# KevinSpevak/openVO

Measured on AMD Instinct MI355X. Metric: stereo frame-pairs/sec (1280x720), higher is better.
Workload: dtype int16

## Files before the change

### openvo_amd/csrc/sgbm.hip

```cpp
#include "vo_internal.h"
#include <stdlib.h>
#include <algorithm>
#include <type_traits>

typedef short s16x2 __attribute__((ext_vector_type(2)));
typedef unsigned short u16x2 __attribute__((ext_vector_type(2)));

#define MAXC 0x7FFF
#define MAXC2 0x7FFF7FFFu
#define D2_EMPTY 0x7FFFFFFF

__device__ __forceinline__ s16x2 as_s(uint32_t v) { return __builtin_bit_cast(s16x2, v); }
__device__ __forceinline__ uint32_t as_u(s16x2 v) { return __builtin_bit_cast(uint32_t, v); }
__device__ __forceinline__ uint32_t pk_min(uint32_t a, uint32_t b) { return as_u(__builtin_elementwise_min(as_s(a), as_s(b))); }
__device__ __forceinline__ uint32_t pk_max(uint32_t a, uint32_t b) { return as_u(__builtin_elementwise_max(as_s(a), as_s(b))); }
__device__ __forceinline__ uint32_t pk_add(uint32_t a, uint32_t b) { return as_u(as_s(a) + as_s(b)); }
__device__ __forceinline__ uint32_t pk_sub(uint32_t a, uint32_t b) { return as_u(as_s(a) - as_s(b)); }
__device__ __forceinline__ uint32_t pk_add_sat(uint32_t a, uint32_t b) { return as_u(__builtin_elementwise_add_sat(as_s(a), as_s(b))); }
__device__ __forceinline__ uint32_t pk_sub_sat_u(uint32_t a, uint32_t b)
{
    return __builtin_bit_cast(uint32_t, __builtin_elementwise_sub_sat(__builtin_bit_cast(u16x2, a), __builtin_bit_cast(u16x2, b)));
}
__device__ __forceinline__ uint32_t pk_shr2(uint32_t a)
{
// ... 23 lines not shown
};

__device__ __forceinline__ int chan_val(const uint8_t* img, int W, int H, int x, int y, int c, int ft)
{
    if (x <= 0 || x >= W - 1) return ft;
    const uint8_t* r0 = img + (size_t)y * W;
    if (c == 1) return r0[x];
    const uint8_t* rn = y > 0 ? r0 - W : r0;
    const uint8_t* rs = y < H - 1 ? r0 + W : r0;
    int g = (r0[x + 1] - r0[x - 1]) * 2 + rn[x + 1] - rn[x - 1] + rs[x + 1] - rs[x - 1];
    return min(max(g, -ft), ft) + ft;
}

__device__ __forceinline__ void chan_bounds(const uint8_t* img, int W, int H, int x, int y, int c, int ft,
                                            int& v, int& lo, int& hi)
{
    v = chan_val(img, W, H, x, y, c, ft);
    int vl = x > 0 ? (v + chan_val(img, W, H, x - 1, y, c, ft)) / 2 : v;
    int vr = x < W - 1 ? (v + chan_val(img, W, H, x + 1, y, c, ft)) / 2 : v;
    lo = min(min(vl, vr), v);
    hi = max(max(vl, vr), v);
}

__global__ void k_sgbm_planes(const uint8_t* __restrict__ L, const uint8_t* __restrict__ R, int W, int H,
                              int ft, uint32_t* __restrict__ PL, uint32_t* __restrict__ PR, int* __restrict__ d2key,
                              int* __restrict__ sw_ctl, int sw_ctl_words, uint32_t* __restrict__ c_dummy, int dummy_words, uint32_t P2_2,
                              uint8_t* __restrict__ keepL, uint8_t* __restrict__ keepR)
{
    const int x = blockIdx.x * blockDim.x + threadIdx.x;
    for (int y = blockIdx.y; y < H; y += gridDim.y) {
    if (y == 1 && blockIdx.x == 0 && (int)threadIdx.x < dummy_words) c_dummy[threadIdx.x] = P2_2;
    if (y == 0 && blockIdx.x == 0)
        for (int i = threadIdx.x; i < sw_ctl_words; i += blockDim.x) sw_ctl[i] = 0;
    if (x >= W) return;
    size_t i = (size_t)y * W + x, plane = (size_t)W * H;
    if (keepL) { keepL[i] = L[i]; keepR[i] = R[i]; }
    if (d2key) d2key[i] = D2_EMPTY;
    for (int c = 0; c < 2; c++) {
        int v, lo, hi;
        chan_bounds(L, W, H, x, y, c, ft, v, lo, hi);
        PL[i * 2 + c] = (uint32_t)v | ((uint32_t)lo << 8) | ((uint32_t)hi << 16);
        int v1 = 0, lo1 = 0, hi1 = 0;
        chan_bounds(R, W, H, x, y, c, ft, v, lo, hi);
        if (x > 0) chan_bounds(R, W, H, x - 1, y, c, ft, v1, lo1, hi1);
        PR[(size_t)(c * 3 + 0) * plane + i] = (uint32_t)v | ((uint32_t)v1 << 16);
        PR[(size_t)(c * 3 + 1) * plane + i] = (uint32_t)lo | ((uint32_t)lo1 << 16);
        PR[(size_t)(c * 3 + 2) * plane + i] = (uint32_t)hi | ((uint32_t)hi1 << 16);
    }
    }
}

// ... 16 lines not shown
        if (c == 1) m = (m >> 2) & 0x3FFF3FFFu;
        acc = pk_add(acc, m);
    }
    return acc;
}

__device__ __forceinline__ uint32_t bt_regs(uint32_t lw0, uint32_t lw1, const uint32_t* V)
{
    uint32_t acc = 0;
#pragma unroll
    for (int c = 0; c < 2; c++) {
        const uint32_t lw = c ? lw1 : lw0;
        const uint32_t U = pk_rep(lw & 255), U0 = pk_rep((lw >> 8) & 255), U1 = pk_rep((lw >> 16) & 255);
        const uint32_t c0 = pk_sub_sat_u(U, V[c * 3 + 2]) | pk_sub_sat_u(V[c * 3 + 1], U);
        const uint32_t c1 = pk_sub_sat_u(V[c * 3 + 0], U1) | pk_sub_sat_u(U0, V[c * 3 + 0]);
        uint32_t m = pk_min(c0, c1);
        if (c == 1) m = pk_shr2(m);
        acc = pk_add(acc, m);
    }
    return acc;
}

template <int XT, int SW2>
__global__ void __launch_bounds__(128) k_sgbm_cost_sweep(const uint32_t* __restrict__ PL, const uint32_t* __restrict__ PR,
                                                        SgbmGeom g, int TY, int16_t* __restrict__ C)
{
    constexpr int WIN = 2 * SW2 + 1, NC = XT + 2 * SW2;
    constexpr bool RING_REGS = WIN <= 5;
    extern __shared__ uint32_t s_ring[];
    uint32_t ringv[RING_REGS ? WIN : 1][XT];
    uint32_t* const ring = s_ring + (size_t)(threadIdx.x >> 6) * WIN * XT * 64 + (threadIdx.x & 63);
    const int lane = threadIdx.x & 63, wv = threadIdx.x >> 6;
    const int dpl = threadIdx.x;
    const bool pad = 2 * dpl >= g.D;
    const int gx = (g.W1 + XT - 1) / XT, total = gx * ((g.H + TY - 1) / TY);
    const int chunk = (total + 7) >> 3, tile = (int)(blockIdx.x & 7) * chunk + (int)(blockIdx.x >> 3);
    if (tile >= total) return;
    const int tbx = tile % gx, tby = tile / gx;
    const int xa = tbx * XT, ya = tby * TY;
    const size_t plane = (size_t)g.W * g.H;
    const int yend = min(ya + TY, g.H);
    const int nrows = (yend - ya) + 2 * SW2;
    const int lane0_d = 2 * 64 * wv;
    const int krun = min(lane, NC - 1);
    const int xrun = min(max(xa - SW2 + krun, 0), g.W1 - 1) + g.minX1;
    const int prun = max(xrun - g.minD - lane0_d, 0);
    const int pown = max(-g.minD - 2 * (pad ? 0 : dpl), -(1 << 28));

    uint32_t acc[XT];
// ... 148 lines not shown
                if (rr >= WIN) acc[j] = pk_sub(acc[j], ringv[slot][j]);
                acc[j] = pk_add(acc[j], s);
                ringv[slot][j] = s;
            } else {
                uint32_t* cell = ring + (size_t)(slot * XT + j) * 64;
                if (rr >= WIN) acc[j] = pk_sub(acc[j], *cell);
                acc[j] = pk_add(acc[j], s);
                *cell = s;
            }
        }
        if (rr >= WIN - 1) {
            const int y = ya + rr - (WIN - 1);
#pragma unroll
            for (int j = 0; j < XT; j++) {
                const int x1 = xa + j;
                if (x1 < g.W1 && 2 * dpl < g.Dp)
                    *(uint32_t*)(C + ((size_t)y * g.W1 + x1) * g.Dp + 2 * dpl) = pad ? MAXC2 : acc[j];
            }
        }
    }
    }
}

__global__ void k_sgbm_cost_generic(const uint32_t* __restrict__ PL, const uint32_t* __restrict__ PR,
                                    SgbmGeom g, int16_t* __restrict__ C)
{
    const int dpl = threadIdx.x;
    if (2 * dpl >= g.Dp) return;
    const bool pad = 2 * dpl >= g.D;
    const int dp = pad ? 0 : dpl;
    const int x1 = blockIdx.x, y = blockIdx.y;
    const size_t plane = (size_t)g.W * g.H;
    const int pbase = g.minX1 - g.minD - 2 * dp;
    uint32_t acc = pk_rep(g.P2);
    for (int j = -g.SW2; j <= g.SW2; j++) {
        int r = min(max(y + j, 0), g.H - 1);
        for (int i = -g.SW2; i <= g.SW2; i++) {
            int xe = min(max(x1 + i, 0), g.W1 - 1);
            acc = pk_add(acc, bt_pair(PL, PR, plane, g.W, r, xe + g.minX1, xe + pbase));
        }
    }
    *(uint32_t*)(C + ((size_t)y * g.W1 + x1) * g.Dp + 2 * dpl) = pad ? MAXC2 : acc;
}

template <int NP>
struct LV { uint32_t r[NP]; };

template <int NP>
__device__ __forceinline__ LV<NP> lv_load(const int16_t* p)
// ... 1008 lines not shown
static int ensure_S(vo_ctx* ctx, int vols)
{
    if (ctx->ws->S_vols >= vols) return VO_OK;
    if (ctx->ws->S) (void)hipFree(ctx->ws->S);
    ctx->ws->S = nullptr; ctx->ws->S_vols = 0;
    VO_HIP(ctx, hipMalloc((void**)&ctx->ws->S, ctx->vol_cells * sizeof(int16_t) * vols + 256));
    ctx->ws->S_vols = vols;
    return VO_OK;
}

static_assert(VO_MAX_SWEEP_GROUP == DG_MAXJOBS, "include/vo355.h promises what one sweep launch carries");
struct SweepGroup {
    typedef int (*Launch)(vo_ctx*, const DiagJobs&, const SgbmGeom&);
    typedef int (*WeLaunch)(vo_ctx*, const WeJobs&, int, const SgbmGeom&);
    struct Member {
        int engine;
        hipStream_t stream;
        FrameSlot* f;
        int w, h;
        SgbmGeom g;
        DiagJob job;
        WeJob we;
        PostJob post;
    };
    Launch launch = nullptr;
    WeLaunch we_launch = nullptr;
    int nstrips = 0;
    int n = 0;
    hipStream_t lane = nullptr;
    Member m[DG_MAXJOBS];
    bool want_defer = false, did_defer = false;
    Member cand;
    Launch cand_launch = nullptr;
    WeLaunch cand_we_launch = nullptr;
    int cand_nstrips = 0;
};

template <int NP>
static int we2_launch_jobs(vo_ctx* ctx, const WeJobs& jobs, int n, const SgbmGeom& g)
{
    const dim3 grid(n, div_up(div_up(g.H, 4), 2));
    if (g.D != g.Dp) hipLaunchKernelGGL((k_sgbm_we2<NP, true>), grid, dim3(256), 0, ctx->stream, jobs, g, ctx->dump);
    else hipLaunchKernelGGL((k_sgbm_we2<NP, false>), grid, dim3(256), 0, ctx->stream, jobs, g, ctx->dump);
    VO_CHECK_LAUNCH(ctx);
    return VO_OK;
}
// ... 53 lines not shown
            G->cand_nstrips = jobs.nstrips;
            G->did_defer = true;
            return VO_OK;
        }
    }
    return diag_launch_jobs<NP, PAD, NWC, REV, WTA>(ctx, jobs, g);
}

template <int NP, bool REV, bool WTA>
static int launch_diag(vo_ctx* ctx, const SgbmGeom& g, const int16_t* in1, int16_t* sout, int* ctl)
{
    const bool pad = g.D != g.Dp;
    if constexpr (NP <= 4) {
        const int nwc = ctx->tune_diag_nwc ? ctx->tune_diag_nwc : (ctx->cur_engine >= 0 ? 11 : 7);
        if (nwc == 15)
            return pad ? launch_diag_k<NP, true, 15, REV, WTA>(ctx, g, in1, sout, ctl) : launch_diag_k<NP, false, 15, REV, WTA>(ctx, g, in1, sout, ctl);
        if (nwc == 11)
            return pad ? launch_diag_k<NP, true, 11, REV, WTA>(ctx, g, in1, sout, ctl) : launch_diag_k<NP, false, 11, REV, WTA>(ctx, g, in1, sout, ctl);
    }

    return pad ? launch_diag_k<NP, true, 7, REV, WTA>(ctx, g, in1, sout, ctl) : launch_diag_k<NP, false, 7, REV, WTA>(ctx, g, in1, sout, ctl);
}

template <int NP>
static int launch_agg(vo_ctx* ctx, const SgbmGeom& g, const PathPlan& plan, size_t vol)
{
    const bool pad = g.D != g.Dp;
    const bool hh = plan.n_dirs == 8;
    int rc;
    if (g.ur < 100) {
        if ((rc = ensure_S(ctx, 3))) return rc;
        int16_t* const Swe = ctx->ws->S;
        int16_t* const Srev = ctx->ws->S + vol;
        int16_t* const ck = ctx->ws->S + 2 * vol;
        int* const ctlA = ctx->ws->sw_ctl;
        int* const ctlB = ctx->ws->sw_ctl + ctx->sw_ctl_words / 2;
        const bool cut = g.W1 % 16 == 0 && g.W1 >= 32 && !(ctx->tune_diag_dbg & 8);
        SweepGroup* const G = ctx->grp;
        const bool defer_we = cut && G && G->want_defer && !hh && !(ctx->tune_diag_dbg & 16);
        if (G) G->cand_we_launch = nullptr;
        {
            StageTimer t(ctx, VO_T_SGBM_AGG, defer_we ? 0 : 1);
            if (ctx->tune_diag_dbg & 8) {
            } else if (cut) {
                WeJobs wj;
                memset(&wj, 0, sizeof(wj));
                wj.j[0].C = ctx->ws->C; wj.j[0].Swe = Swe; wj.j[0].ckpt = ck;
                if (defer_we) {
                    G->cand.we = wj.j[0];
                    G->cand_we_launch = &we2_launch_jobs<NP>;
                } else if ((rc = we2_launch_jobs<NP>(ctx, wj, 1, g))) return rc;
            } else if (g.W1 % 8 == 0 && g.W1 >= 16) {
                const int nw = div_up(g.H, 4);
                if (pad) hipLaunchKernelGGL((k_sgbm_we<NP, true>), dim3(div_up(nw, 4)), dim3(256), 0, ctx->stream, ctx->ws->C, Swe, ck, g, ctx->dump);
                else hipLaunchKernelGGL((k_sgbm_we<NP, false>), dim3(div_up(nw, 4)), dim3(256), 0, ctx->stream, ctx->ws->C, Swe, ck, g, ctx->dump);
            } else {
                PathPlan pp = plan;
                pp.n_dirs = 1;
                pp.sx[0] = 1; pp.sy[0] = 0; pp.nlines[0] = g.H;
                pp.first_wave[0] = 0;
                for (int k = 0; k < VO_MAX_DIRS; k++) pp.first_wave[k + 1] = div_up(g.H, 4);
                for (int k = 1; k < VO_MAX_DIRS; k++) pp.sx[k] = pp.sy[k] = pp.nlines[k] = 0;
// ... 25 lines not shown
        else hipLaunchKernelGGL((k_sgbm_paths<NP, PF, false>), dim3(div_up(nwaves, 4)), dim3(256), 0, ctx->stream, ctx->ws->C, ctx->ws->S, vol, g, plan, ctx->dump);
        VO_CHECK_LAUNCH(ctx);
    }
    {
        StageTimer t(ctx, VO_T_SGBM_WTA);
        const size_t sh = (size_t)16 * g.Dp * sizeof(int16_t);
        const long long npix = (long long)g.W1 * g.H;
        hipLaunchKernelGGL((k_sgbm_wta<NP>), dim3((unsigned)((npix + 15) / 16)), dim3(256), sh, ctx->stream, ctx->ws->S, vol, plan.n_dirs,
                           g, ctx->ws->disp_tmp, ctx->ws->ccl_size);
        VO_CHECK_LAUNCH(ctx);
    }
    ctx->last_paths = plan.n_dirs;
    ctx->last_schedule = VO_SCHED_UNFUSED;
    return VO_OK;
}

static int sgbm_run_impl(vo_ctx* ctx, FrameSlot& f, int w, int h, const uint8_t* srcL, const uint8_t* srcR);
static int sgbm_post(vo_ctx* ctx, FrameSlot& f, int w, int h, const SgbmGeom& g);
static PostJob post_job(const vo_ctx* ctx, const FrameSlot& f);
static int sgbm_post_launch(vo_ctx* ctx, const PostJobs& jobs, int n, const SgbmGeom& g, bool rows);
static uint32_t pk_rep_host(int v) { return (uint32_t)(v & 0xFFFF) * 0x00010001u; }
static int post_rows_per_block(int w) { return std::min(6, (int)(150 * 1024 / ((size_t)w * 6)) - 2); }

static int sgbm_run_done(vo_ctx* ctx)
{
    if (ctx->ws == &ctx->main_ws && ctx->ws->done) {
        VO_HIP(ctx, hipEventRecord(ctx->ws->done, ctx->stream));
        ctx->ws->done_valid = true;
        ctx->ws->done_on_engine0 = false;
        ctx->ws->done_lane = nullptr;
    }
    return VO_OK;
}

int sgbm_run(vo_ctx* ctx, FrameSlot& f, int w, int h, const uint8_t* srcL, const uint8_t* srcR, bool* deferred)
{
    int rc;
    if (deferred) *deferred = false;
    if (ctx->cur_engine < 0 && sweep_group_has_engine(ctx, 0) && (rc = sweep_group_close(ctx, VO_GRP_CONSUMER))) return rc;
    const bool shared = ctx->ws == &ctx->main_ws;
    if (shared && ctx->ws->done_valid && !(ctx->cur_engine == 0 && ctx->ws->done_on_engine0) && !(ctx->ws->done_lane && ctx->ws->done_lane == ctx->stream)) VO_HIP(ctx, hipStreamWaitEvent(ctx->stream, ctx->ws->done, 0));
    if (++ctx->sweep_gen_next <= 0) ctx->sweep_gen_next = 1;
    f.disp_gen = ctx->sweep_gen_next;
    const bool defer = deferred && ctx->cur_engine >= 0 && sweep_group_size(ctx) > 1 && ctx->sg.set && ctx->sg.ur < 100 && ctx->sg.mode == 0 &&
                       ctx->ws_alt[ctx->cur_engine].mid != nullptr;
    if (defer) {
        if (!ctx->grp) ctx->grp = new SweepGroup();
        ctx->grp->want_defer = true;
        ctx->grp->did_defer = false;
    }
    rc = sgbm_run_impl(ctx, f, w, h, srcL, srcR);
    if (defer) {
        SweepGroup* const G = ctx->grp;
        G->want_defer = false;
        if (!rc && G->did_defer) {
            G->did_defer = false;
            if (G->n > 0 && (G->n >= DG_MAXJOBS || G->launch != G->cand_launch || G->we_launch != G->cand_we_launch || G->nstrips != G->cand_nstrips ||
                             memcmp(&G->m[0].g, &G->cand.g, sizeof(SgbmGeom))) &&
                (rc = sweep_group_close(ctx, VO_GRP_OTHER)))
                return rc;
            SweepGroup::Member& m = G->m[G->n++];
            m = G->cand;
            m.engine = ctx->cur_engine; m.stream = ctx->stream; m.f = &f; m.w = w; m.h = h;
            if (G->n == 1) G->lane = stream_is_lane(ctx, ctx->stream) ? ctx->stream : nullptr;
            m.post = post_job(ctx, f);
            G->launch = G->cand_launch; G->we_launch = G->cand_we_launch; G->nstrips = G->cand_nstrips;
            f.in_group = true;
            *deferred = true;
            return VO_OK;
        }
    }
    if (int rcd = sgbm_run_done(ctx)) return rcd;
    return rc;
}

hipStream_t dense_stream(const vo_ctx* ctx, int engine)
{
    if (!lane_mode(ctx) || !ctx->sg.set || ctx->sg.ur >= 100 || ctx->sg.mode != 0) return ctx->la_stream[engine];
    const SweepGroup* const G = ctx->grp;
    return G && G->n > 0 && G->lane ? G->lane : ctx->lane[ctx->lane_next];
}

bool sweep_group_has_engine(const vo_ctx* ctx, int engine)
{
    if (ctx->grp)
        for (int i = 0; i < ctx->grp->n; i++)
            if (ctx->grp->m[i].engine == engine) return true;
    return false;
}
int sweep_group_members(const vo_ctx* ctx) { return ctx->grp ? ctx->grp->n : 0; }
void sweep_group_free(vo_ctx* ctx) { delete ctx->grp; ctx->grp = nullptr; }
// ... 61 lines not shown
    G->n = 0;
    for (int i = 0; i < n; i++) G->m[i].f->in_group = false;
    ctx->grp_closed[why]++;
    int rc = VO_OK;
    {
        MemberScope scope(ctx);
        SweepGroup::Member& last = G->m[n - 1];
        scope.enter(last.engine);
        hipStream_t const lane = G->lane;
        G->lane = nullptr;
        if (lane) {
            ctx->stream = lane;
            ctx->lane_next = lane == ctx->lane[0] ? 1 : 0;
        }
        DiagJobs jobs;
        WeJobs we;
        PostJobs post;
        memset(&jobs, 0, sizeof(jobs));
        memset(&we, 0, sizeof(we));
        memset(&post, 0, sizeof(post));
        jobs.n = n; jobs.nstrips = G->nstrips;
        jobs.j[0] = last.job; we.j[0] = last.we; post.j[0] = last.post;
        bool main_member = last.engine == 0;
        for (int i = 0; i + 1 < n && !rc; i++) {
            jobs.j[i + 1] = G->m[i].job; we.j[i + 1] = G->m[i].we; post.j[i + 1] = G->m[i].post;
            main_member |= G->m[i].engine == 0;
            const vo_ctx::SgbmWs& a = ctx->ws_alt[G->m[i].engine];
            if (lane && G->m[i].stream == lane) continue;
            if (!a.mid_valid || hipStreamWaitEvent(ctx->stream, a.mid, 0) != hipSuccess) rc = vo_fail(ctx, VO_E_HIP, "sweep group: waiting for a member's early stages failed");
        }
        if (!rc && G->we_launch) {
            StageTimer t(ctx, VO_T_SGBM_AGG, n);
            rc = G->we_launch(ctx, we, n, last.g);
        }
        if (!rc) {
            StageTimer t(ctx, VO_T_SGBM_WTA, n);
            rc = G->launch(ctx, jobs, last.g);
        }
        const bool post_here = post_rows_per_block(last.g.W) >= 1;
        if (!rc && post_here) {
            if (!(ctx->tune_diag_dbg & 32)) {
                StageTimer t(ctx, VO_T_SGBM_POST, n);
                rc = sgbm_post_launch(ctx, post, n, last.g, true);
            }
            if (!rc && main_member && ctx->main_ws.done) {
                if (hipEventRecord(ctx->main_ws.done, ctx->stream) == hipSuccess) { ctx->main_ws.done_valid = true; ctx->main_ws.done_on_engine0 = false; ctx->main_ws.done_lane = lane; }
// ... 58 lines not shown
    int maxX1 = w + (e.minD < 0 ? e.minD : 0);
    g.W1 = maxX1 - g.minX1;
    g.invalid16 = (e.minD - 1) * 16;
    const int n = w * h;
    if (g.W1 <= 0) {
        if (srcL) {
            VO_HIP(ctx, hipMemcpyAsync(f.left, srcL, (size_t)n, hipMemcpyDeviceToDevice, ctx->stream));
            VO_HIP(ctx, hipMemcpyAsync(f.right, srcR, (size_t)n, hipMemcpyDeviceToDevice, ctx->stream));
        }
        std::vector<int16_t> inv((size_t)n, (int16_t)g.invalid16);
        VO_HIP(ctx, hipMemcpyAsync(d_disp, inv.data(), (size_t)n * 2, hipMemcpyHostToDevice, ctx->stream));
        VO_HIP(ctx, hipStreamSynchronize(ctx->stream));
        ctx->last_cells = 0;
        return VO_OK;
    }
    const size_t vol = (size_t)g.W1 * h * g.Dp;
    if (vol > ctx->vol_cells || e.D > 256)
        return vo_fail(ctx, VO_E_CAP, "cost volume %zu cells exceeds the capacity given to vo_create (or D > 256)", vol);
    if (((size_t)g.W1 * h + 1) * g.Dp * 2 >= 0xFFFFFF00ull)
        return vo_fail(ctx, VO_E_CAP, "cost volume of %zu bytes exceeds the 4 GiB a volume kernel addresses", ((size_t)g.W1 * h + 1) * g.Dp * 2);
    const PathPlan plan = make_plan(g, e.mode);
    ctx->last_cells = (int64_t)g.W1 * h * g.D;
    {
        StageTimer t(ctx, VO_T_SGBM_COST);
        const int dbg = ctx->tune_diag_dbg;
        hipLaunchKernelGGL(k_sgbm_planes, dim3(div_up(w, 256), std::min(h, 128)), dim3(256), 0, ctx->stream, dL, dR, w, h, g.ftzero,
                           ctx->ws->planesL, ctx->ws->planesR, (g.ur >= 100 || post_rows_per_block(w) < 1) ? ctx->ws->ccl_size : nullptr, ctx->ws->sw_ctl, ctx->sw_ctl_words,
                           (uint32_t*)(ctx->ws->C + vol), g.Dp / 2, pk_rep_host(g.P2), srcL ? f.left : nullptr, srcL ? f.right : nullptr);
        const int bx = ((g.Dp / 2 + 63) / 64) * 64;
        const int TY = ctx->tune_sweep_ty;
        const int nw = bx / 64;
#define LAUNCH_SWEEP(XT, SW)                                                                                                   \
    hipLaunchKernelGGL((k_sgbm_cost_sweep<XT, SW>), dim3(8 * div_up(div_up(g.W1, XT) * div_up(h, TY), 8)), dim3(bx),            \
                       (size_t)nw * (((2 * SW + 1) <= 5 ? 0 : (2 * SW + 1) * XT * 64) + 12 * (64 + (XT + 2 * SW - 1) / 2)) * 4, ctx->stream, ctx->ws->planesL, ctx->ws->planesR, g, TY, ctx->ws->C)
        if (dbg & 4) {
        } else
        switch (g.SW2) {
            case 0: LAUNCH_SWEEP(8, 0); break;
            case 1: LAUNCH_SWEEP(8, 1); break;
            case 2: LAUNCH_SWEEP(8, 2); break;
            case 3: LAUNCH_SWEEP(8, 3); break;
            case 4: LAUNCH_SWEEP(8, 4); break;
            case 5: LAUNCH_SWEEP(8, 5); break;
            default:
                hipLaunchKernelGGL(k_sgbm_cost_generic, dim3(g.W1, h), dim3(bx), 0, ctx->stream, ctx->ws->planesL, ctx->ws->planesR, g, ctx->ws->C);
        }
#undef LAUNCH_SWEEP
        VO_CHECK_LAUNCH(ctx);
    }
    int rc;
    switch (g.Dp / 32) {
        case 1: rc = launch_agg<1>(ctx, g, plan, vol); break;
        case 2: rc = launch_agg<2>(ctx, g, plan, vol); break;
        case 3: rc = launch_agg<3>(ctx, g, plan, vol); break;
        case 4: rc = launch_agg<4>(ctx, g, plan, vol); break;
        case 5: rc = launch_agg<5>(ctx, g, plan, vol); break;
        case 6: rc = launch_agg<6>(ctx, g, plan, vol); break;
        case 7: rc = launch_agg<7>(ctx, g, plan, vol); break;
        default: rc = launch_agg<8>(ctx, g, plan, vol); break;
    }
    if (rc) return rc;
    if (ctx->grp && ctx->grp->did_defer) return VO_OK;
    return sgbm_post(ctx, f, w, h, g);
}

static PostJob post_job(const vo_ctx* ctx, const FrameSlot& f)
{
    PostJob j;
    j.aux0 = ctx->ws->rec; j.aux1 = ctx->ws->rec + (size_t)ctx->max_w * ctx->max_h + 64;
    j.dst = f.disp16;
    j.L = ctx->ws->ccl_label; j.runlen = ctx->ws->ccl_runlen; j.size = ctx->ws->ccl_size;
// ... 54 lines not shown
```

### openvo_amd/csrc/vo_ctx.hip

```cpp
#include <stdarg.h>
#include <stdlib.h>
#include "vo_internal.h"

int vo_fail(vo_ctx* ctx, int code, const char* fmt, ...)
{
    char buf[1024];
    va_list ap;
    va_start(ap, fmt);
    vsnprintf(buf, sizeof(buf), fmt, ap);
    va_end(ap);
    if (ctx) ctx->err = buf;
    return code;
}

static thread_local std::string g_create_err;
static int lanes_ensure(vo_ctx* ctx);

static const size_t ARENA_BASE = 4096;

static void* arena_take(vo_ctx* ctx, size_t bytes)
{
    const size_t need = (bytes + 63) & ~(size_t)63;
    if (ARENA_BASE + ctx->arena_off + need > ctx->pinned_bytes) return nullptr;
    void* p = (char*)ctx->pinned + ARENA_BASE + ctx->arena_off;
// ... 133 lines not shown
    int ndev = 0;
    hipError_t e = hipGetDeviceCount(&ndev);
    if (e != hipSuccess || ndev <= 0) {
        g_create_err = std::string("vo_create: no HIP device available (") + hipGetErrorString(e) +
                       "); libvo355 has no CPU fallback";
        return VO_E_HIP;
    }
    if (device_id < 0 || device_id >= ndev) { g_create_err = "vo_create: bad device id"; return VO_E_ARG; }
    vo_ctx* ctx = new vo_ctx();
    ctx->device = device_id;
    ctx->max_w = max_w; ctx->max_h = max_h; ctx->max_disp = max_disp; ctx->max_kp = max_kp;
    if ((e = hipSetDevice(device_id)) != hipSuccess) { g_create_err = hipGetErrorString(e); delete ctx; return VO_E_HIP; }
    hipDeviceProp_t prop;
    if (hipGetDeviceProperties(&prop, device_id) == hipSuccess) {
        char generic[96];
        snprintf(generic, sizeof(generic), "AMD GPU, %d CUs, %.0f GB", prop.multiProcessorCount, (double)prop.totalGlobalMem / 1e9);
        snprintf(ctx->devname, sizeof(ctx->devname), "%s (%s)", prop.name[0] ? prop.name : generic, prop.gcnArchName);
    }
    if ((e = hipStreamCreateWithFlags(&ctx->stream, hipStreamNonBlocking)) != hipSuccess) { g_create_err = hipGetErrorString(e); delete ctx; return VO_E_HIP; }
    if (const char* e8 = getenv("VO_ENGINES")) { int v = atoi(e8); if (v >= 1 && v <= vo_ctx::MAX_ENGINES) ctx->n_engines = v; }
    if (const char* eq = getenv("GPU_MAX_HW_QUEUES")) { int v = atoi(eq); if (v >= 1) ctx->hw_queues = v; }
    if (const char* eg = getenv("VO_SWEEP_GROUP")) { int v = atoi(eg); if (v >= 1 && v <= VO_MAX_SWEEP_GROUP) ctx->sweep_group_req = v; }
    if (const char* el = getenv("VO_GROUP_LANES")) ctx->lanes_on = atoi(el) != 0;
    if (lanes_ensure(ctx)) { g_create_err = "hipStreamCreate failed (lane streams)"; vo_destroy(ctx); return VO_E_HIP; }
    (void)hipEventCreate(&ctx->ev0);
    (void)hipEventCreate(&ctx->ev1);

    const size_t npx = (size_t)max_w * max_h;
    ctx->kp_cap = max_kp * 2 + 1024;
    for (int s = 0; s <= VO_NUM_SLOTS; s++) {
        FrameSlot& f = ctx->slots[s];
        DALLOC(f.left, npx); DALLOC(f.right, npx); DALLOC(f.disp16, npx);
        (void)hipEventCreateWithFlags(&f.ready, hipEventDisableTiming);
        DALLOC(f.kp_xy, (size_t)ctx->kp_cap * 2); DALLOC(f.kp_size, ctx->kp_cap); DALLOC(f.kp_angle, ctx->kp_cap);
        DALLOC(f.kp_resp, ctx->kp_cap); DALLOC(f.kp_oct, ctx->kp_cap); DALLOC(f.desc, (size_t)ctx->kp_cap * 32);
        DALLOC(f.mono_depth, ctx->kp_cap); DALLOC(f.mono_serial_dev, 16);
        DALLOC(f.kp_xyz, (size_t)ctx->kp_cap * 3); DALLOC(f.kp_disp, ctx->kp_cap); DALLOC(f.kp_rdesc, (size_t)ctx->kp_cap * 32);
        if (dev_zero(f.mono_serial_dev, 64) != hipSuccess) { g_create_err = "clearing a slot's depth serial failed"; vo_destroy(ctx); return VO_E_HIP; }
    }
    {
        FrameSlot& r = ctx->sparse_r;
        DALLOC(r.kp_xy, (size_t)ctx->kp_cap * 2); DALLOC(r.kp_size, ctx->kp_cap); DALLOC(r.kp_angle, ctx->kp_cap);
        DALLOC(r.kp_resp, ctx->kp_cap); DALLOC(r.kp_oct, ctx->kp_cap); DALLOC(r.desc, (size_t)ctx->kp_cap * 32);
        ctx->sp_main.l = &ctx->slots[VO_NUM_SLOTS]; ctx->sp_main.r = &r;
    }
    ctx->stage_bytes = npx * 3;
// ... 348 lines not shown
    return VO_OK;
}

extern "C" int vo_upload_mono(vo_ctx* ctx, int slot, const uint8_t* img, int w, int h, int channels)
{
    int rc = check_slot(ctx, slot);
    if (rc) return rc;
    if (!img || (channels != 1 && channels != 3)) return vo_fail(ctx, VO_E_ARG, "vo_upload_mono: bad argument");
    if (w > ctx->max_w || h > ctx->max_h || w < 16 || h < 16) return vo_fail(ctx, VO_E_CAP, "image %dx%d exceeds context %dx%d", w, h, ctx->max_w, ctx->max_h);
    VO_HIP(ctx, hipSetDevice(ctx->device));
    FrameSlot& f = ctx->slots[slot];
    if ((rc = slot_wait(ctx, f)) || (rc = slot_before_overwrite(ctx, f))) return rc;
    StageTimer t(ctx, VO_T_UPLOAD);
    if ((rc = ingest(ctx, 0, img, w, h, channels, 1, f.left, ctx->stage_in))) return rc;
    f.w = w; f.h = h; f.has_pair = true; f.has_disp = false; f.has_kp = false; f.kp_depth = false; f.sp_pending = false; f.n_kp = 0; f.kp_pending = false;
    return VO_OK;
}

extern "C" int vo_stage_pairs_alloc(vo_ctx* ctx, int n, int w, int h, int channels)
{
    if (!ctx || n <= 0 || (channels != 1 && channels != 3)) return vo_fail(ctx, VO_E_ARG, "vo_stage_pairs_alloc: bad argument");
    if (w > ctx->max_w || h > ctx->max_h || w < 16 || h < 16) return vo_fail(ctx, VO_E_CAP, "image %dx%d exceeds context", w, h);
    VO_HIP(ctx, hipSetDevice(ctx->device));
    if (ctx->staged) { (void)hipFree(ctx->staged); ctx->staged = nullptr; }
    ctx->staged_n = 0;
    const size_t per = (size_t)w * h * channels;
    VO_HIP(ctx, hipMalloc((void**)&ctx->staged, per * 2 * n));
    ctx->staged_n = n; ctx->staged_w = w; ctx->staged_h = h; ctx->staged_ch = channels;
    return VO_OK;
}

extern "C" int vo_stage_pair(vo_ctx* ctx, int index, const uint8_t* left, const uint8_t* right)
{
    if (!ctx || !left || !right || index < 0 || index >= ctx->staged_n) return vo_fail(ctx, VO_E_ARG, "vo_stage_pair: bad index");
    VO_HIP(ctx, hipSetDevice(ctx->device));
    const size_t per = (size_t)ctx->staged_w * ctx->staged_h * ctx->staged_ch;
    VO_HIP(ctx, hipMemcpyAsync(ctx->staged + per * 2 * index, left, per, hipMemcpyHostToDevice, ctx->stream));
    VO_HIP(ctx, hipMemcpyAsync(ctx->staged + per * (2 * index + 1), right, per, hipMemcpyHostToDevice, ctx->stream));
    VO_HIP(ctx, hipStreamSynchronize(ctx->stream));
    return VO_OK;
}

extern "C" int vo_load_staged_pair(vo_ctx* ctx, int slot, int index, int preprocessed)
{
    int rc = check_slot(ctx, slot);
    if (rc) return rc;
    if (index < 0 || index >= ctx->staged_n) return vo_fail(ctx, VO_E_ARG, "vo_load_staged_pair: bad index");
    VO_HIP(ctx, hipSetDevice(ctx->device));
    FrameSlot& f = ctx->slots[slot];
    const int w = ctx->staged_w, h = ctx->staged_h;
    const size_t per = (size_t)w * h * ctx->staged_ch;
    StageTimer t(ctx, VO_T_UPLOAD);
    if ((rc = slot_wait(ctx, f)) || (rc = slot_before_overwrite(ctx, f))) return rc;
    rc = ingest(ctx, 0, ctx->staged + per * 2 * index, w, h, ctx->staged_ch, preprocessed, f.left, ctx->stage_in, hipMemcpyDeviceToDevice);
    if (rc) return rc;
    rc = ingest(ctx, 1, ctx->staged + per * (2 * index + 1), w, h, ctx->staged_ch, preprocessed, f.right, ctx->stage_in, hipMemcpyDeviceToDevice);
    if (rc) return rc;
    f.w = w; f.h = h; f.has_pair = true; f.has_disp = false; f.has_kp = false; f.kp_depth = false; f.sp_pending = false; f.n_kp = 0; f.kp_pending = false;
    return VO_OK;
// ... 871 lines not shown
```

### openvo_amd/csrc/vo_internal.h

```cpp
#pragma once
#include <hip/hip_runtime.h>
#include <stdint.h>
#include <stdio.h>
#include <string.h>
#include <string>
#include <vector>
#include <deque>
#include <thread>
#include <mutex>
#include <condition_variable>
#include "../../include/vo355.h"

#define VO_ORB_LEVELS 8
#define VO_ORB_EDGE 31
#define VO_ORB_HALF_PATCH 15

struct SgbmEff {
    int minD, maxD, D, ur, d12, P1, P2, SW2, SH2, ftzero, minX1, maxX1, W1, invalid16;
    int speckleWindow, speckleRange, mode;
    bool set;
};

struct OrbLevel {
    int w, h;
// ... 63 lines not shown
struct MapSet {
    float* xyz = nullptr;
    uint8_t *desc = nullptr, *rdesc = nullptr;
    int32_t *oct = nullptr, *obs = nullptr, *last = nullptr;
};
struct LandmarkMap {
    bool used = false;
    int capacity = 0, n = 0, cur = 0, view_n = 0;
    int max_serial = -1;
    MapSet set[2];
    int32_t *view_src = nullptr, *d_q = nullptr, *d_t = nullptr;
    uint8_t *claimed = nullptr, *d_mask = nullptr;
    std::vector<uint8_t> seen;
};
void map_free(LandmarkMap& m);

struct vo_ctx {
    int device = 0;
    hipStream_t stream = nullptr;
    static const int MAX_ENGINES = 24;
    hipStream_t la_stream[MAX_ENGINES] = {};
    hipStream_t lane[2] = {nullptr, nullptr};
    bool lanes_on = true;
    bool lane_used = false;
    int lane_next = 0;
    int cur_engine = -1;
    int tune_stagger = -1;
    uint8_t* la_stage[MAX_ENGINES] = {};
    struct SgbmWs {
        uint32_t *planesL = nullptr, *planesR = nullptr;
        int16_t *C = nullptr, *S = nullptr, *disp_tmp = nullptr;
        int32_t *ccl_runlen = nullptr, *ccl_label = nullptr, *ccl_size = nullptr;
        int32_t* rec = nullptr;
        int S_vols = 0;
        uint64_t* sw_bnd = nullptr;
        size_t sw_bnd_bytes = 0;
        int* sw_ctl = nullptr;
        uint32_t sw_tag = 0;
        hipEvent_t done = nullptr;
        bool done_valid = false;
        bool done_on_engine0 = false;
        hipStream_t done_lane = nullptr;
        bool ready = false;
        OrbWs orb;
        uint8_t* pinned = nullptr;
        hipEvent_t h2d_done = nullptr;
// ... 233 lines not shown
{
    int few = VO_SWEEP_GROUP_FEW_QUEUES;
    if (ctx->lanes_on && few > ctx->n_engines / 2) few = ctx->n_engines >= 2 ? ctx->n_engines / 2 : 1;
    int b = ctx->sweep_group_req > 0 ? ctx->sweep_group_req : (ctx->hw_queues >= ctx->n_engines + 4 ? 1 : few);
    return b < ctx->n_engines ? b : ctx->n_engines;
}
static inline bool lane_mode(const vo_ctx* ctx) { return ctx->lanes_on && ctx->lane[0] && ctx->lane[1] && sweep_group_size(ctx) > 1; }
static inline int pose_stream_count(const vo_ctx* ctx)
{
    int n = ctx->n_pose_streams;
    if (!ctx->pose_streams_env && ctx->lane_used && lane_mode(ctx) && n > ctx->hw_queues - 3) n = ctx->hw_queues - 3 > 1 ? ctx->hw_queues - 3 : 1;
    return n;
}
static inline bool stream_is_lane(const vo_ctx* ctx, hipStream_t s) { return s && (s == ctx->lane[0] || s == ctx->lane[1]); }
static inline hipError_t engine_streams_sync(const vo_ctx* ctx)
{
    for (int k = 0; k < 2; k++)
        if (ctx->lane[k]) { const hipError_t e = hipStreamSynchronize(ctx->lane[k]); if (e != hipSuccess) return e; }
    for (int k = 0; k < vo_ctx::MAX_ENGINES; k++)
        if (ctx->la_stream[k]) { const hipError_t e = hipStreamSynchronize(ctx->la_stream[k]); if (e != hipSuccess) return e; }
    return hipSuccess;
}
int sweep_group_close(vo_ctx* ctx, int why);
int engine_behind_chain(vo_ctx* ctx, int engine);
int engine_enter(vo_ctx* ctx, int engine, hipStream_t target);
hipStream_t dense_stream(const vo_ctx* ctx, int engine);
bool sweep_group_has_engine(const vo_ctx* ctx, int engine);
int sweep_group_members(const vo_ctx* ctx);
void sweep_group_free(vo_ctx* ctx);
static inline int sweep_group_close_for(vo_ctx* ctx, const FrameSlot& f) { return f.in_group ? sweep_group_close(ctx, VO_GRP_CONSUMER) : VO_OK; }
int slot_health(vo_ctx* ctx, const FrameSlot& f, int slot);
int orb_prepare_tables(vo_ctx* ctx, int w, int h);
int orb_run(vo_ctx* ctx, FrameSlot* fs, const uint8_t* d_img, int img_stride, int w, int h,
            int nfeatures, int mask_mode, const int16_t* d_disp16, int disp_stride, int min_d16,
            int max_d16, const uint8_t* d_mask, int mask_stride);
#define VO_KNN_SPLITS 16
static inline size_t match_dist_bytes(int kp_cap)
{
    const size_t capq = ((size_t)kp_cap + 63) & ~(size_t)63;
    return capq * 8 + (size_t)VO_KNN_SPLITS * capq * 8 + (capq / 64 + 1) * 4 + capq * 4 + 256;
}
static inline uint32_t* match_colmin(int32_t* d_dist, int kp_cap)
{
    const size_t capq = ((size_t)kp_cap + 63) & ~(size_t)63;
    return (uint32_t*)((uint8_t*)d_dist + capq * 8 + (size_t)VO_KNN_SPLITS * capq * 8 + (capq / 64 + 1) * 4);
}
// ... 61 lines not shown
```

Baseline: 2182.

## Batch SGBM planes and cost-volume launches across sweep-group frames

The planes and cost-sweep kernels now take an array of per-frame jobs indexed by a grid dimension. When frames are deferred into a sweep group on a lane stream, each frame's front-end work is queued, then launched as one batched kernel pair once enough frames are pending or the group closes. This cuts per-frame launch count and lets several frames fill the GPU together. The cost is extra deferral bookkeeping, flush points in the staging APIs, and an abandon path for the group when a batched launch fails.

```diff
diff --git a/openvo_amd/csrc/sgbm.hip b/openvo_amd/csrc/sgbm.hip
--- a/openvo_amd/csrc/sgbm.hip
+++ b/openvo_amd/csrc/sgbm.hip
@@ -69,11 +69,29 @@
     hi = max(max(vl, vr), v);
 }
 
-__global__ void k_sgbm_planes(const uint8_t* __restrict__ L, const uint8_t* __restrict__ R, int W, int H,
-                              int ft, uint32_t* __restrict__ PL, uint32_t* __restrict__ PR, int* __restrict__ d2key,
-                              int* __restrict__ sw_ctl, int sw_ctl_words, uint32_t* __restrict__ c_dummy, int dummy_words, uint32_t P2_2,
-                              uint8_t* __restrict__ keepL, uint8_t* __restrict__ keepR)
-{
+struct FrontJob {
+    const uint8_t *L, *R;
+    uint32_t *planesL, *planesR;
+    int* d2key;
+    int* sw_ctl;
+    uint32_t* dummy;
+    uint8_t *keepL, *keepR;
+    int16_t* C;
+};
+struct FrontJobs { FrontJob j[VO_MAX_SWEEP_GROUP]; };
+
+__global__ void k_sgbm_planes(FrontJobs jobs, int W, int H, int ft, int sw_ctl_words, int dummy_words, uint32_t P2_2)
+{
+    const FrontJob& J = jobs.j[blockIdx.z];
+    const uint8_t* __restrict__ const L = J.L;
+    const uint8_t* __restrict__ const R = J.R;
+    uint32_t* __restrict__ const PL = J.planesL;
+    uint32_t* __restrict__ const PR = J.planesR;
+    int* __restrict__ const d2key = J.d2key;
+    int* __restrict__ const sw_ctl = J.sw_ctl;
+    uint32_t* __restrict__ const c_dummy = J.dummy;
+    uint8_t* __restrict__ const keepL = J.keepL;
+    uint8_t* __restrict__ const keepR = J.keepR;
     const int x = blockIdx.x * blockDim.x + threadIdx.x;
     for (int y = blockIdx.y; y < H; y += gridDim.y) {
     if (y == 1 && blockIdx.x == 0 && (int)threadIdx.x < dummy_words) c_dummy[threadIdx.x] = P2_2;
@@ -136,9 +154,12 @@
 }
 
 template <int XT, int SW2>
-__global__ void __launch_bounds__(128) k_sgbm_cost_sweep(const uint32_t* __restrict__ PL, const uint32_t* __restrict__ PR,
-                                                        SgbmGeom g, int TY, int16_t* __restrict__ C)
-{
+__global__ void __launch_bounds__(128) k_sgbm_cost_sweep(FrontJobs jobs, SgbmGeom g, int TY)
+{
+    const FrontJob& J = jobs.j[blockIdx.y];
+    const uint32_t* __restrict__ const PL = J.planesL;
+    const uint32_t* __restrict__ const PR = J.planesR;
+    int16_t* __restrict__ const C = J.C;
     constexpr int WIN = 2 * SW2 + 1, NC = XT + 2 * SW2;
     constexpr bool RING_REGS = WIN <= 5;
     extern __shared__ uint32_t s_ring[];
@@ -333,9 +354,12 @@
     }
 }
 
-__global__ void k_sgbm_cost_generic(const uint32_t* __restrict__ PL, const uint32_t* __restrict__ PR,
-                                    SgbmGeom g, int16_t* __restrict__ C)
-{
+__global__ void k_sgbm_cost_generic(FrontJobs jobs, SgbmGeom g)
+{
+    const FrontJob& J = jobs.j[blockIdx.z];
+    const uint32_t* __restrict__ const PL = J.planesL;
+    const uint32_t* __restrict__ const PR = J.planesR;
+    int16_t* __restrict__ const C = J.C;
     const int dpl = threadIdx.x;
     if (2 * dpl >= g.Dp) return;
     const bool pad = 2 * dpl >= g.D;
@@ -1390,6 +1414,8 @@
         DiagJob job;
         WeJob we;
         PostJob post;
+        FrontJob front;
+        bool front_pending;
     };
     Launch launch = nullptr;
     WeLaunch we_launch = nullptr;
@@ -1489,6 +1515,21 @@
     return pad ? launch_diag_k<NP, true, 7, REV, WTA>(ctx, g, in1, sout, ctl) : launch_diag_k<NP, false, 7, REV, WTA>(ctx, g, in1, sout, ctl);
 }
 
+static bool we2_geometry(const vo_ctx* ctx, const SgbmGeom& g) { return g.W1 % 16 == 0 && g.W1 >= 32 && !(ctx->tune_diag_dbg & 8); }
+
+static bool run_defers_we(const vo_ctx* ctx, const SgbmGeom& g, bool hh)
+{
+    const SweepGroup* const G = ctx->grp;
+    return G && G->want_defer && g.ur < 100 && g.W1 > 0 && we2_geometry(ctx, g) && !hh && !(ctx->tune_diag_dbg & 16);
+}
+
+static bool run_defers_front(const vo_ctx* ctx, const SgbmGeom& g, bool hh)
+{
+    if (ctx->front_batch < 2 || ctx->cur_engine < 0 || (ctx->tune_diag_dbg & 4) || !run_defers_we(ctx, g, hh)) return false;
+    if (!lane_mode(ctx) || !stream_is_lane(ctx, ctx->stream)) return false;
+    return ctx->grp->n == 0 || ctx->grp->lane == ctx->stream;
+}
+
 template <int NP>
 static int launch_agg(vo_ctx* ctx, const SgbmGeom& g, const PathPlan& plan, size_t vol)
 {
@@ -1502,9 +1543,9 @@
         int16_t* const ck = ctx->ws->S + 2 * vol;
         int* const ctlA = ctx->ws->sw_ctl;
         int* const ctlB = ctx->ws->sw_ctl + ctx->sw_ctl_words / 2;
-        const bool cut = g.W1 % 16 == 0 && g.W1 >= 32 && !(ctx->tune_diag_dbg & 8);
+        const bool cut = we2_geometry(ctx, g);
         SweepGroup* const G = ctx->grp;
-        const bool defer_we = cut && G && G->want_defer && !hh && !(ctx->tune_diag_dbg & 16);
+        const bool defer_we = run_defers_we(ctx, g, hh);
         if (G) G->cand_we_launch = nullptr;
         {
             StageTimer t(ctx, VO_T_SGBM_AGG, defer_we ? 0 : 1);
@@ -1576,6 +1617,80 @@
 static uint32_t pk_rep_host(int v) { return (uint32_t)(v & 0xFFFF) * 0x00010001u; }
 static int post_rows_per_block(int w) { return std::min(6, (int)(150 * 1024 / ((size_t)w * 6)) - 2); }
 
+static int front_launch(vo_ctx* ctx, const FrontJobs& jobs, int n, const SgbmGeom& g)
+{
+    const int w = g.W, h = g.H;
+    hipLaunchKernelGGL(k_sgbm_planes, dim3(div_up(w, 256), std::min(h, 128), n), dim3(256), 0, ctx->stream, jobs, w, h, g.ftzero,
+                       ctx->sw_ctl_words, g.Dp / 2, pk_rep_host(g.P2));
+    const int bx = ((g.Dp / 2 + 63) / 64) * 64;
+    const int TY = ctx->tune_sweep_ty;
+    const int nw = bx / 64;
+#define LAUNCH_SWEEP(XT, SW)                                                                                                   \
+    hipLaunchKernelGGL((k_sgbm_cost_sweep<XT, SW>), dim3(8 * div_up(div_up(g.W1, XT) * div_up(h, TY), 8), n), dim3(bx),         \
+                       (size_t)nw * (((2 * SW + 1) <= 5 ? 0 : (2 * SW + 1) * XT * 64) + 12 * (64 + (XT + 2 * SW - 1) / 2)) * 4, ctx->stream, jobs, g, TY)
+    if (ctx->tune_diag_dbg & 4) {
+    } else
+    switch (g.SW2) {
+        case 0: LAUNCH_SWEEP(8, 0); break;
+        case 1: LAUNCH_SWEEP(8, 1); break;
+        case 2: LAUNCH_SWEEP(8, 2); break;
+        case 3: LAUNCH_SWEEP(8, 3); break;
+        case 4: LAUNCH_SWEEP(8, 4); break;
+        case 5: LAUNCH_SWEEP(8, 5); break;
+        default:
+            hipLaunchKernelGGL(k_sgbm_cost_generic, dim3(g.W1, h, n), dim3(bx), 0, ctx->stream, jobs, g);
+    }
+#undef LAUNCH_SWEEP
+    VO_CHECK_LAUNCH(ctx);
+    return VO_OK;
+}
+
+static int sweep_group_launch_fronts(vo_ctx* ctx, SweepGroup* G, int n, hipStream_t lane)
+{
+    FrontJobs fj;
+    memset(&fj, 0, sizeof(fj));
+    int k = 0;
+    for (int i = 0; i < n; i++)
+        if (G->m[i].front_pending) { fj.j[k++] = G->m[i].front; G->m[i].front_pending = false; }
+    if (k == 0) return VO_OK;
+    hipStream_t const s0 = ctx->stream;
+    ctx->stream = lane;
+    int rc;
+    {
+        StageTimer t(ctx, VO_T_SGBM_COST, k);
+        rc = front_launch(ctx, fj, k, G->m[0].g);
+    }
+    ctx->stream = s0;
+    return rc;
+}
+
+static void sweep_group_abandon(vo_ctx* ctx)
+{
+    SweepGroup* const G = ctx->grp;
+    for (int i = 0; i < G->n; i++) {
+        FrameSlot& f = *G->m[i].f;
+        f.in_group = false; f.kp_pending = false; f.has_pair = false; f.has_disp = false;
+        if (f.counted && ctx->inflight > 0) ctx->inflight--;
+        f.counted = false;
+    }
+    G->n = 0;
+    G->lane = nullptr;
+}
+
+int sweep_group_flush_fronts(vo_ctx* ctx, bool wait)
+{
+    SweepGroup* const G = ctx->grp;
+    if (!G || G->n == 0 || !G->lane) return VO_OK;
+    bool any = false;
+    for (int i = 0; i < G->n; i++) any |= G->m[i].front_pending;
+    if (!any) return VO_OK;
+    (void)hipSetDevice(ctx->device);
+    hipStream_t const lane = G->lane;
+    if (int rc = sweep_group_launch_fronts(ctx, G, G->n, lane)) { sweep_group_abandon(ctx); return rc; }
+    if (wait) VO_HIP(ctx, hipStreamSynchronize(lane));
+    return VO_OK;
+}
+
 static int sgbm_run_done(vo_ctx* ctx)
 {
     if (ctx->ws == &ctx->main_ws && ctx->ws->done) {
@@ -1602,6 +1717,7 @@
         if (!ctx->grp) ctx->grp = new SweepGroup();
         ctx->grp->want_defer = true;
         ctx->grp->did_defer = false;
+        ctx->grp->cand.front_pending = false;
     }
     rc = sgbm_run_impl(ctx, f, w, h, srcL, srcR);
     if (defer) {
@@ -1621,6 +1737,12 @@
             G->launch = G->cand_launch; G->we_launch = G->cand_we_launch; G->nstrips = G->cand_nstrips;
             f.in_group = true;
             *deferred = true;
+            int pending = 0;
+            for (int i = 0; i < G->n; i++) pending += G->m[i].front_pending ? 1 : 0;
+            if (pending >= ctx->front_batch && G->lane && (rc = sweep_group_launch_fronts(ctx, G, G->n, G->lane))) {
+                sweep_group_abandon(ctx);
+                return rc;
+            }
             return VO_OK;
         }
     }
@@ -1728,6 +1850,7 @@
         jobs.n = n; jobs.nstrips = G->nstrips;
         jobs.j[0] = last.job; we.j[0] = last.we; post.j[0] = last.post;
         bool main_member = last.engine == 0;
+        if (lane) rc = sweep_group_launch_fronts(ctx, G, n, lane);
         for (int i = 0; i + 1 < n && !rc; i++) {
             jobs.j[i + 1] = G->m[i].job; we.j[i + 1] = G->m[i].we; post.j[i + 1] = G->m[i].post;
             main_member |= G->m[i].engine == 0;
@@ -1832,31 +1955,21 @@
     const PathPlan plan = make_plan(g, e.mode);
     ctx->last_cells = (int64_t)g.W1 * h * g.D;
     {
-        StageTimer t(ctx, VO_T_SGBM_COST);
-        const int dbg = ctx->tune_diag_dbg;
-        hipLaunchKernelGGL(k_sgbm_planes, dim3(div_up(w, 256), std::min(h, 128)), dim3(256), 0, ctx->stream, dL, dR, w, h, g.ftzero,
-                           ctx->ws->planesL, ctx->ws->planesR, (g.ur >= 100 || post_rows_per_block(w) < 1) ? ctx->ws->ccl_size : nullptr, ctx->ws->sw_ctl, ctx->sw_ctl_words,
-                           (uint32_t*)(ctx->ws->C + vol), g.Dp / 2, pk_rep_host(g.P2), srcL ? f.left : nullptr, srcL ? f.right : nullptr);
-        const int bx = ((g.Dp / 2 + 63) / 64) * 64;
-        const int TY = ctx->tune_sweep_ty;
-        const int nw = bx / 64;
-#define LAUNCH_SWEEP(XT, SW)                                                                                                   \
-    hipLaunchKernelGGL((k_sgbm_cost_sweep<XT, SW>), dim3(8 * div_up(div_up(g.W1, XT) * div_up(h, TY), 8)), dim3(bx),            \
-                       (size_t)nw * (((2 * SW + 1) <= 5 ? 0 : (2 * SW + 1) * XT * 64) + 12 * (64 + (XT + 2 * SW - 1) / 2)) * 4, ctx->stream, ctx->ws->planesL, ctx->ws->planesR, g, TY, ctx->ws->C)
-        if (dbg & 4) {
-        } else
-        switch (g.SW2) {
-            case 0: LAUNCH_SWEEP(8, 0); break;
-            case 1: LAUNCH_SWEEP(8, 1); break;
-            case 2: LAUNCH_SWEEP(8, 2); break;
-            case 3: LAUNCH_SWEEP(8, 3); break;
-            case 4: LAUNCH_SWEEP(8, 4); break;
-            case 5: LAUNCH_SWEEP(8, 5); break;
-            default:
-                hipLaunchKernelGGL(k_sgbm_cost_generic, dim3(g.W1, h), dim3(bx), 0, ctx->stream, ctx->ws->planesL, ctx->ws->planesR, g, ctx->ws->C);
-        }
-#undef LAUNCH_SWEEP
-        VO_CHECK_LAUNCH(ctx);
+        FrontJobs fj;
+        memset(&fj, 0, sizeof(fj));
+        FrontJob& j = fj.j[0];
+        j.L = dL; j.R = dR; j.planesL = ctx->ws->planesL; j.planesR = ctx->ws->planesR;
+        j.d2key = (g.ur >= 100 || post_rows_per_block(w) < 1) ? ctx->ws->ccl_size : nullptr;
+        j.sw_ctl = ctx->ws->sw_ctl; j.dummy = (uint32_t*)(ctx->ws->C + vol);
+        j.keepL = srcL ? f.left : nullptr; j.keepR = srcL ? f.right : nullptr;
+        j.C = ctx->ws->C;
+        if (run_defers_front(ctx, g, plan.n_dirs == 8)) {
+            ctx->grp->cand.front = j;
+            ctx->grp->cand.front_pending = true;
+        } else {
+            StageTimer t(ctx, VO_T_SGBM_COST);
+            if (int rcf = front_launch(ctx, fj, 1, g)) return rcf;
+        }
     }
     int rc;
     switch (g.Dp / 32) {
diff --git a/openvo_amd/csrc/vo_ctx.hip b/openvo_amd/csrc/vo_ctx.hip
--- a/openvo_amd/csrc/vo_ctx.hip
+++ b/openvo_amd/csrc/vo_ctx.hip
@@ -179,6 +179,7 @@
     if (const char* eq = getenv("GPU_MAX_HW_QUEUES")) { int v = atoi(eq); if (v >= 1) ctx->hw_queues = v; }
     if (const char* eg = getenv("VO_SWEEP_GROUP")) { int v = atoi(eg); if (v >= 1 && v <= VO_MAX_SWEEP_GROUP) ctx->sweep_group_req = v; }
     if (const char* el = getenv("VO_GROUP_LANES")) ctx->lanes_on = atoi(el) != 0;
+    if (const char* ef = getenv("VO_GROUP_FRONTS")) { int v = atoi(ef); if (v >= 0) ctx->front_batch = v > VO_MAX_SWEEP_GROUP ? VO_MAX_SWEEP_GROUP : v; }
     if (lanes_ensure(ctx)) { g_create_err = "hipStreamCreate failed (lane streams)"; vo_destroy(ctx); return VO_E_HIP; }
     (void)hipEventCreate(&ctx->ev0);
     (void)hipEventCreate(&ctx->ev1);
@@ -573,6 +574,7 @@
     if (!ctx || n <= 0 || (channels != 1 && channels != 3)) return vo_fail(ctx, VO_E_ARG, "vo_stage_pairs_alloc: bad argument");
     if (w > ctx->max_w || h > ctx->max_h || w < 16 || h < 16) return vo_fail(ctx, VO_E_CAP, "image %dx%d exceeds context", w, h);
     VO_HIP(ctx, hipSetDevice(ctx->device));
+    if (int rc = sweep_group_flush_fronts(ctx, true)) return rc;
     if (ctx->staged) { (void)hipFree(ctx->staged); ctx->staged = nullptr; }
     ctx->staged_n = 0;
     const size_t per = (size_t)w * h * channels;
@@ -586,6 +588,7 @@
     if (!ctx || !left || !right || index < 0 || index >= ctx->staged_n) return vo_fail(ctx, VO_E_ARG, "vo_stage_pair: bad index");
     VO_HIP(ctx, hipSetDevice(ctx->device));
     const size_t per = (size_t)ctx->staged_w * ctx->staged_h * ctx->staged_ch;
+    if (int rc = sweep_group_flush_fronts(ctx, true)) return rc;
     VO_HIP(ctx, hipMemcpyAsync(ctx->staged + per * 2 * index, left, per, hipMemcpyHostToDevice, ctx->stream));
     VO_HIP(ctx, hipMemcpyAsync(ctx->staged + per * (2 * index + 1), right, per, hipMemcpyHostToDevice, ctx->stream));
     VO_HIP(ctx, hipStreamSynchronize(ctx->stream));
diff --git a/openvo_amd/csrc/vo_internal.h b/openvo_amd/csrc/vo_internal.h
--- a/openvo_amd/csrc/vo_internal.h
+++ b/openvo_amd/csrc/vo_internal.h
@@ -109,6 +109,7 @@
     hipStream_t la_stream[MAX_ENGINES] = {};
     hipStream_t lane[2] = {nullptr, nullptr};
     bool lanes_on = true;
+    int front_batch = 8;
     bool lane_used = false;
     int lane_next = 0;
     int cur_engine = -1;
@@ -388,6 +389,7 @@
     return hipSuccess;
 }
 int sweep_group_close(vo_ctx* ctx, int why);
+int sweep_group_flush_fronts(vo_ctx* ctx, bool wait);
 int engine_behind_chain(vo_ctx* ctx, int engine);
 int engine_enter(vo_ctx* ctx, int engine, hipStream_t target);
 hipStream_t dense_stream(const vo_ctx* ctx, int engine);
```

After: 2367, median of 6. 1.08x the previous value.
